# victorramirez952/tomography_3d_reconstructor

Hardware: NVIDIA B200
Metric: Gvoxels/s mask-stack->mesh+volume (higher is better)
Workload: dtype u8 -> bit-packed u32 (topology), f64 field taps -> f32 vertices

## Files before the change

tomography_3d_reconstructor_b200/csrc/t3d_mc.cu:

```cuda
#include "mc_tables.h"
#include "mc33_tables.h"
#include "t3d.h"
#include "t3d_field.cuh"

__device__ __align__(16) const int8_t g_tri_table[256][T3D_MC_ROW] = {T3D_TRI_TABLE_ROWS};
static const int8_t h_tri_table[256][T3D_MC_ROW] = {T3D_TRI_TABLE_ROWS};

struct McLuts {
    uint8_t ntri[256];
};
#define MC_AMB 0x80u
__constant__ McLuts c_luts;

__device__ const int8_t g33_rows[T3D_MC33_NROWS][T3D_MC33_ROW] = {T3D_MC33_TRI_ROWS};
__device__ const uint8_t g33_ntri[T3D_MC33_NROWS] = {T3D_MC33_NTRI_VALUES};
__device__ const uint16_t g33_base[256] = {T3D_MC33_BASE_VALUES};
__device__ const uint8_t g33_k[256] = {T3D_MC33_K_VALUES};
__device__ const uint8_t g33_faces[256][6] = {T3D_MC33_FACES_VALUES};
__device__ const unsigned long long g33_need[256] = {T3D_MC33_NEED_VALUES};
__device__ const uint8_t g33_pol[256] = {T3D_MC33_POL_VALUES};
__device__ const int8_t g33_sign[256] = {T3D_MC33_SIGN_VALUES};
__device__ const uint8_t g33_cyc[6][4] = {T3D_MC33_FACE_CYCLE_VALUES};
static const uint16_t h33_base[256] = {T3D_MC33_BASE_VALUES};

// ... 277 lines not shown
            int z, y;
            const WordMasks m = load_masks(g, row, w, z, y);
            int delta = 0;
            for (uint32_t a = m.act; a;) {
                const int b = __ffs(a) - 1;
                a &= a - 1;
                const int cs = cube_case(m, b);
                const uint32_t c = c_luts.ntri[cs];
                if (!(c & MC_AMB)) continue;
                delta += (int)g33_ntri[mc33_resolve(fld, z, y, (w << 5) + b, cs)] - (int)(c & 0x7fu);
                ++na;
            }
            aw_cnt[3 * (int64_t)n_active + k] += (uint32_t)delta;
        };
        const int64_t n4 = ((uintptr_t)aw_idx & 15) ? 0 : (n >> 2), stride = (int64_t)gridDim.x * blockDim.x, t0 = (int64_t)blockIdx.x * blockDim.x + threadIdx.x;
        for (int64_t c = t0; c < n4; c += stride) {
            const uint4 v = reinterpret_cast<const uint4*>(aw_idx)[c];
            if (!((v.x | v.y | v.z | v.w) & AW_AMB)) continue;
            if (v.x & AW_AMB) fix_word(4 * c, v.x);
            if (v.y & AW_AMB) fix_word(4 * c + 1, v.y);
            if (v.z & AW_AMB) fix_word(4 * c + 2, v.z);
            if (v.w & AW_AMB) fix_word(4 * c + 3, v.w);
        }
        for (int64_t k = 4 * n4 + t0; k < n; k += stride) {
            const uint32_t iraw = aw_idx[k];
            if (iraw & AW_AMB) fix_word(k, iraw);
        }
        if (na) atomicAdd(n_ambiguous, (unsigned long long)na);
    }
}

static unsigned amb_grid(uint32_t n) { const unsigned want = (n + 127) / 128, cap = (unsigned)T3D_NUM_SMS * 8; return want < cap ? (want ? want : 1) : cap; }

struct EmitArgs {
    Grid g;
    McField fld;
    const uint32_t* ballots;
    const uint32_t* chunkbase;
    const uint32_t* aw_idx;
    const uint32_t* aw_base;
    uint32_t cap_active;
    const unsigned long long* sizes;
    uint32_t cap_verts, cap_faces;
    unsigned long long* vkeys;
    int32_t* faces;
};

__device__ __forceinline__ uint32_t active_rank(const EmitArgs& a, uint32_t row, int w)
{
    const int64_t c = (int64_t)row * a.g.ncr + (w >> 5);
    return a.chunkbase[c] + __popc(a.ballots[c] & ((1u << (w & 31)) - 1u));
}

__device__ __forceinline__ uint32_t lt_mask(int b) { return b >= 32 ? 0xffffffffu : ((1u << b) - 1u); }

__device__ __forceinline__ unsigned long long vkey(int axis, int z, int y, int x)
{
    return (unsigned long long)axis | ((unsigned long long)x << 2) | ((unsigned long long)y << 22) | ((unsigned long long)z << 42);
}

template <int PARTS, int AMB>
__global__ void __launch_bounds__(128) k_mc_emit(EmitArgs a)
{
    __shared__ __align__(16) int8_t s_tri[256][T3D_MC_ROW];
    __shared__ uint32_t s_base[12][128];
    __shared__ uint32_t s_mask[12][128];
    __shared__ uint32_t s_next[4][128];
    if (AMB == 1) {
        int any = 0;
        uint32_t nw_ = a.cap_active;
        if (a.sizes[0] < nw_) nw_ = (uint32_t)a.sizes[0];
        for (uint32_t k = blockIdx.x * blockDim.x + threadIdx.x; k < nw_; k += gridDim.x * blockDim.x) any |= (int)(a.aw_idx[k] >> 31);
        if (!__syncthreads_or(any)) return;
    }
    if (PARTS & 2) {
        const int4* src = reinterpret_cast<const int4*>(&g_tri_table[0][0]);
        int4* dst = reinterpret_cast<int4*>(&s_tri[0][0]);
        for (int i = threadIdx.x; i < 256; i += blockDim.x) {
            dst[i] = src[i];
            if (c_luts.ntri[i] & MC_AMB) s_tri[i][T3D_MC_ROW - 1] = -2;
        }
        __syncthreads();
    }
    const uint32_t tid = threadIdx.x;
    uint32_t n_words = a.cap_active;
    if (a.sizes[0] < n_words) n_words = (uint32_t)a.sizes[0];
    const uint32_t offY = (uint32_t)a.sizes[1], offZ = (uint32_t)(a.sizes[1] + a.sizes[2]);
    if (a.sizes[1] + a.sizes[2] + a.sizes[3] > a.cap_verts || a.sizes[4] > a.cap_faces) return;
    auto emit_word = [&](const uint32_t k, const uint32_t iraw) {
    const uint32_t i = iraw & AW_MASK;
    const uint32_t row = i / (uint32_t)a.g.nws;
    const int w = (int)(i - row * (uint32_t)a.g.nws);
    int z, y;
    const WordMasks m = load_masks(a.g, row, w, z, y);
    const int64_t NA = a.cap_active;
    const uint32_t bX00 = a.aw_base[k], bY0 = offY + a.aw_base[NA + k], bZ0 = offZ + a.aw_base[2 * NA + k];
    uint32_t pT = a.aw_base[3 * NA + k];
    const int x0 = w << 5;

    if (PARTS & 1) {
        uint32_t id = bX00;
        for (uint32_t q = m.X00; q;) { const int b = __ffs(q) - 1; q &= q - 1; a.vkeys[id++] = vkey(2, z, y, x0 + b); }
        id = bY0;
        for (uint32_t q = m.Y0; q;) { const int b = __ffs(q) - 1; q &= q - 1; a.vkeys[id++] = vkey(1, z, y, x0 + b); }
        id = bZ0;
        for (uint32_t q = m.Z0; q;) { const int b = __ffs(q) - 1; q &= q - 1; a.vkeys[id++] = vkey(0, z, y, x0 + b); }
    }
    if (!(PARTS & 2) || !m.act) return;
    if (AMB == 0 && (iraw & AW_AMB)) return;

    const uint32_t Hs = (uint32_t)a.g.Hs;
    uint32_t bX01 = 0, bX10 = 0, bX11 = 0, bY1 = 0, bZ1 = 0;
    if (m.X01 | m.Z1) {
        const uint32_t r = active_rank(a, row + 1, w);
        bX01 = a.aw_base[r];
        bZ1 = offZ + a.aw_base[2 * NA + r];
    }
    if (m.X10 | m.Y1) {
        const uint32_t r = active_rank(a, row + Hs, w);
        bX10 = a.aw_base[r];
        bY1 = offY + a.aw_base[NA + r];
    }
    if (m.X11) bX11 = a.aw_base[active_rank(a, row + Hs + 1, w)];
    uint32_t nY0 = 0, nY1 = 0, nZ0 = 0, nZ1 = 0;
    if ((m.act >> 31) & 1u) {
        const uint32_t v1 = (m.a00 >> 31) & 1u, v2 = (m.a01 >> 31) & 1u, v5 = (m.a10 >> 31) & 1u, v6 = (m.a11 >> 31) & 1u;
        if (v1 != v2) nY0 = offY + a.aw_base[NA + active_rank(a, row, w + 1)];
        if (v5 != v6) nY1 = offY + a.aw_base[NA + active_rank(a, row + Hs, w + 1)];
        if (v1 != v5) nZ0 = offZ + a.aw_base[2 * NA + active_rank(a, row, w + 1)];
        if (v2 != v6) nZ1 = offZ + a.aw_base[2 * NA + active_rank(a, row + 1, w + 1)];
    }
    s_base[0][tid] = bX00; s_mask[0][tid] = m.X00;
    s_base[1][tid] = bY0;  s_mask[1][tid] = m.Y0;
    s_base[2][tid] = bX01; s_mask[2][tid] = m.X01;
    s_base[3][tid] = bY0;  s_mask[3][tid] = m.Y0;
    s_base[4][tid] = bX10; s_mask[4][tid] = m.X10;
    s_base[5][tid] = bY1;  s_mask[5][tid] = m.Y1;
    s_base[6][tid] = bX11; s_mask[6][tid] = m.X11;
    s_base[7][tid] = bY1;  s_mask[7][tid] = m.Y1;
    s_base[8][tid] = bZ0;  s_mask[8][tid] = m.Z0;
    s_base[9][tid] = bZ0;  s_mask[9][tid] = m.Z0;
    s_base[10][tid] = bZ1; s_mask[10][tid] = m.Z1;
    s_base[11][tid] = bZ1; s_mask[11][tid] = m.Z1;
    s_next[0][tid] = nY0; s_next[1][tid] = nY1; s_next[2][tid] = nZ0; s_next[3][tid] = nZ1;

    auto vertex_id = [&](int b, int e) -> uint32_t {
        const uint32_t at_next = (0x622u >> e) & 1u;
        uint32_t id = s_base[e][tid] + __popc(s_mask[e][tid] & (at_next ? lt_mask(b + 1) : lt_mask(b)));
        if (b == 31 && at_next) id = s_next[((e >> 2) & 1) + 2 * ((e >> 3) & 1) + ((e >> 3) & 1) * ((e >> 1) & 1)][tid];
        return id;
    };
    auto emit_classic = [&](int b, int cs) {
        const int4 trow = *reinterpret_cast<const int4*>(s_tri[cs]);
        const uint32_t tw[4] = {(uint32_t)trow.x, (uint32_t)trow.y, (uint32_t)trow.z, (uint32_t)trow.w};
        auto edge_at = [&](int t) -> int { return (int)(int8_t)((tw[t >> 2] >> ((t & 3) * 8)) & 0xffu); };
        for (int t = 0; t < 15; t += 3) {
            const int e0 = edge_at(t);
            if (e0 < 0) break;
            uint32_t vid[3];
#pragma unroll
            for (int c = 0; c < 3; ++c) vid[c] = vertex_id(b, (c == 0) ? e0 : edge_at(t + c));
            int32_t* f = a.faces + 3 * (int64_t)pT;
            f[0] = (int32_t)vid[2]; f[1] = (int32_t)vid[1]; f[2] = (int32_t)vid[0];
            ++pT;
        }
    };
    if constexpr (AMB == 0) {
        for (uint32_t q = m.act; q;) {
            const int b = __ffs(q) - 1;
            q &= q - 1;
            emit_classic(b, cube_case(m, b));
        }
    } else {
    for (uint32_t q = m.act; q;) {
        const int b = __ffs(q) - 1;
        q &= q - 1;
        const int cs = cube_case(m, b);
        if ((uint8_t)s_tri[cs][T3D_MC_ROW - 1] != 0xfeu) { emit_classic(b, cs); continue; }
        const int r = mc33_resolve(a.fld, z, y, x0 + b, cs);
        const int8_t* row = g33_rows[r];
        const int n3 = 3 * (int)g33_ntri[r];
        for (int t = 0; t < n3; t += 3) {
            int32_t* f = a.faces + 3 * (int64_t)pT;
            f[0] = (int32_t)vertex_id(b, row[t + 2]); f[1] = (int32_t)vertex_id(b, row[t + 1]); f[2] = (int32_t)vertex_id(b, row[t]);
            ++pT;
        }
    }
    }
    };
    if (AMB == 1) {
        for (uint32_t k = blockIdx.x * blockDim.x + tid; k < n_words; k += gridDim.x * blockDim.x) {
            const uint32_t iraw = a.aw_idx[k];
            if (iraw & AW_AMB) emit_word(k, iraw);
        }
    } else {
        const uint32_t k = blockIdx.x * blockDim.x + tid;
        if (k < n_words) emit_word(k, a.aw_idx[k]);
    }
}

struct VertexArgs {
    OccView occ;
    const float* field;
    double level;
    const unsigned long long* vkeys;
    int x_off;
    int z_offset;
    float shift;
    const double* cum;
    const double* adj;
    int n_cum;
    double mm_y, mm_x;
    int scale_f64;
    float* verts;
};

template <int AXIS>
__device__ __forceinline__ void vertex_body(const VertexArgs& p, const ZLut& zlut, uint32_t id)
{
    const unsigned long long key = p.vkeys[id];
    const int x = (int)((key >> 2) & 0xfffffu) - p.x_off, y = (int)((key >> 22) & 0xfffffu), z = (int)(key >> 42);
    float fa, fb;
    if (p.field) {
        const int64_t i = ((int64_t)z * p.occ.H + y) * p.occ.W + x;
        fa = p.field[i];
        fb = p.field[i + (AXIS == 0 ? (int64_t)p.occ.H * p.occ.W : AXIS == 1 ? p.occ.W : 1)];
    } else {
        edge_field_values<AXIS>(p.occ, zlut, z, y, x, fa, fb);
    }
    const double va = (double)fa - p.level, vb = (double)fb - p.level;
    const double wa = __ddiv_rn(1.0, __dadd_rn(MC33_EPS, fabs(va)));
    const double wb = __ddiv_rn(1.0, __dadd_rn(MC33_EPS, fabs(vb)));
    const double frac = __ddiv_rn(wb, __dadd_rn(wa, wb));
    double pz = (double)(z + p.z_offset), py = (double)y, px = (double)x;
    if (AXIS == 0) pz = __dadd_rn(pz, frac); else if (AXIS == 1) py = __dadd_rn(py, frac); else px = __dadd_rn(px, frac);
    float fz = __fsub_rn(__double2float_rn(pz), p.shift);
    float fy = __fsub_rn(__double2float_rn(py), p.shift);
    float fx = __fsub_rn(__double2float_rn(px), p.shift);
    if (p.n_cum > 0) {
        if (fz < 0.0f) fz = 0.0f;
        else if (fz >= (float)(p.n_cum - 1)) fz = __double2float_rn(p.cum[p.n_cum - 1]);
        else {
            const float fl = floorf(fz);
            const int lo = (int)fl;
            const float fr = __fsub_rn(fz, fl);
            const int ai = min(lo, p.n_cum - 2);
            fz = __double2float_rn(__dadd_rn(p.cum[lo], __dmul_rn((double)fr, p.adj[ai])));
        }
    }
    if (p.scale_f64) {
        fy = __double2float_rn(__dmul_rn((double)fy, p.mm_y));
        fx = __double2float_rn(__dmul_rn((double)fx, p.mm_x));
    } else {
        fy = __fmul_rn(fy, __double2float_rn(p.mm_y));
        fx = __fmul_rn(fx, __double2float_rn(p.mm_x));
    }
    float* o = p.verts + 3 * (int64_t)id;
    o[0] = fz; o[1] = fy; o[2] = fx;
}

__global__ void __launch_bounds__(128) k_mc_vertices_all(VertexArgs p, const unsigned long long* __restrict__ sizes, uint32_t cap_verts,
                                                         int which)
{
    __shared__ ZLut zlut;
    fill_zlut(p.occ, zlut);
    __syncthreads();
    const unsigned long long nx = sizes[1], ny = sizes[2], nz = sizes[3];
    if (nx + ny + nz > cap_verts) return;
    uint32_t t = blockIdx.x * blockDim.x + threadIdx.x;
    if (which & 1) {
        if (t < nx) { vertex_body<2>(p, zlut, t); return; }
        t -= (uint32_t)nx;
    }
    if (which & 2) {
        if (t < ny) { vertex_body<1>(p, zlut, (uint32_t)nx + t); return; }
        t -= (uint32_t)ny;
    }
    if ((which & 4) && t < nz) vertex_body<0>(p, zlut, (uint32_t)(nx + ny) + t);
}

static int make_grid(Grid& g, const void* sign_bits, int Zs, int Hs, int Ws, int z_begin, int z_end, const char* who)
{
    if (Zs <= 0 || Hs <= 0 || Ws <= 0) { t3d_set_error("%s: empty volume", who); return 2; }
    if (z_end < 0 || z_end > Zs) z_end = Zs;
    if (z_begin < 0 || z_begin >= z_end) { t3d_set_error("%s: empty plane range", who); return 2; }
    g.z_begin = z_begin; g.z_end = z_end;
    g.sign = (const uint32_t*)sign_bits;
    g.Zs = Zs; g.Hs = Hs; g.Ws = Ws; g.nws = t3d_wpr(Ws);
    g.ncr = (g.nws + 31) >> 5;
    g.n_rows = (uint32_t)((int64_t)Zs * Hs);
    g.n_words = (int64_t)Zs * Hs * g.nws;
    if (g.n_words >= ((int64_t)1 << 31)) { t3d_set_error("%s: more than 2^31 words in one device slab", who); return 2; }
    return 0;
}
// ... 36 lines not shown
    T3D_CHECK_LAUNCH("t3d_mc_words_dev");
    t3d_count_launches(3);
    return 0;
}

extern "C" int t3d_mc_words_dev(const void* sign_bits, int Zs, int Hs, int Ws, int z_begin, int z_end, const void* ballots_u32,
                                const void* chunkbase_u32, uint32_t cap_active, const void* sizes_u64, void* aw_idx_u32,
                                void* aw_cnt_u32, void* n_ambiguous_u64, const t3d_mc_field* mc_field, void* stream)
{
    return mc_words_dev_impl(mc_field_from_abi(mc_field), sign_bits, Zs, Hs, Ws, z_begin, z_end, ballots_u32, chunkbase_u32, cap_active,
                             sizes_u64, aw_idx_u32, aw_cnt_u32, n_ambiguous_u64, stream);
}

static int mc_emit_dev_impl(const McField& fld, const void* sign_bits, int Zs, int Hs, int Ws, int z_begin, int z_end,
                            const void* ballots_u32, const void* chunkbase_u32, const void* aw_idx_u32, const void* aw_base_u32,
                            uint32_t cap_active, const void* sizes_u64, uint32_t cap_verts, uint32_t cap_faces, void* vkeys_u64,
                            void* faces_i32, int parts, void* stream)
{
    EmitArgs a;
    if (int rc = make_grid(a.g, sign_bits, Zs, Hs, Ws, z_begin, z_end, "t3d_mc_emit_dev")) return rc;
    if (ensure_luts()) return 1;
    if (cap_active == 0) return 0;
    a.fld = fld;
    a.ballots = (const uint32_t*)ballots_u32;
    a.chunkbase = (const uint32_t*)chunkbase_u32;
    a.aw_idx = (const uint32_t*)aw_idx_u32;
    a.aw_base = (const uint32_t*)aw_base_u32;
    a.cap_active = cap_active;
    a.sizes = (const unsigned long long*)sizes_u64;
    a.cap_verts = cap_verts;
    a.cap_faces = cap_faces;
    a.vkeys = (unsigned long long*)vkeys_u64;
    a.faces = (int32_t*)faces_i32;
    const unsigned ge = (cap_active + 127) / 128;
    int launches = 1;
    if ((parts & 3) == 1) k_mc_emit<1, 0><<<ge, 128, 0, (cudaStream_t)stream>>>(a);
    else if ((parts & 3) == 2) {
        k_mc_emit<2, 0><<<ge, 128, 0, (cudaStream_t)stream>>>(a);
        k_mc_emit<2, 1><<<amb_grid(cap_active), 128, 0, (cudaStream_t)stream>>>(a);
        launches = 2;
    } else k_mc_emit<3, 2><<<ge, 128, 0, (cudaStream_t)stream>>>(a);
    T3D_CHECK_LAUNCH("t3d_mc_emit_dev");
    t3d_count_launches(launches);
    return 0;
}

extern "C" int t3d_mc_emit_dev(const void* sign_bits, int Zs, int Hs, int Ws, int z_begin, int z_end, const void* ballots_u32,
                               const void* chunkbase_u32, const void* aw_idx_u32, const void* aw_base_u32, uint32_t cap_active,
                               const void* sizes_u64, uint32_t cap_verts, uint32_t cap_faces, void* vkeys_u64, void* faces_i32,
                               int parts, const t3d_mc_field* mc_field, void* stream)
{
    return mc_emit_dev_impl(mc_field_from_abi(mc_field), sign_bits, Zs, Hs, Ws, z_begin, z_end, ballots_u32, chunkbase_u32, aw_idx_u32,
                            aw_base_u32, cap_active, sizes_u64, cap_verts, cap_faces, vkeys_u64, faces_i32, parts, stream);
}

int t3d_mc_words_view_dev(const OccView& view, int x_off, const void* sign_bits, int Zs, int Hs, int Ws, int z_begin, int z_end,
                          const void* ballots_u32, const void* chunkbase_u32, uint32_t cap_active, const void* sizes_u64,
                          void* aw_idx_u32, void* aw_cnt_u32, void* n_ambiguous_u64, void* stream)
{
    McField f;
    f.occ = view; f.field = nullptr; f.level = 0.5; f.x_off = x_off; f.mode = 1;
    return mc_words_dev_impl(f, sign_bits, Zs, Hs, Ws, z_begin, z_end, ballots_u32, chunkbase_u32, cap_active, sizes_u64, aw_idx_u32,
                             aw_cnt_u32, n_ambiguous_u64, stream);
}

int t3d_mc_emit_view_dev(const OccView& view, int x_off, const void* sign_bits, int Zs, int Hs, int Ws, int z_begin, int z_end,
                         const void* ballots_u32, const void* chunkbase_u32, const void* aw_idx_u32, const void* aw_base_u32,
                         uint32_t cap_active, const void* sizes_u64, uint32_t cap_verts, uint32_t cap_faces, void* vkeys_u64,
                         void* faces_i32, int parts, void* stream)
{
    McField f;
    f.occ = view; f.field = nullptr; f.level = 0.5; f.x_off = x_off; f.mode = 1;
    return mc_emit_dev_impl(f, sign_bits, Zs, Hs, Ws, z_begin, z_end, ballots_u32, chunkbase_u32, aw_idx_u32, aw_base_u32, cap_active,
                            sizes_u64, cap_verts, cap_faces, vkeys_u64, faces_i32, parts, stream);
}

// ... 77 lines not shown
```

tomography_3d_reconstructor_b200/csrc/t3d_field.cuh:

```cuda
#pragma once
#include "t3d_common.cuh"

struct OccView {
    const uint32_t* bits;
    int Z, H, W, nw;
    int rs;
    long long ps;
    int pad;
    int Zp, Hp, Wp;
    int gaussian;
    double w0, w1, w2;
};

__device__ __forceinline__ int reflect_idx(int i, int n)
{
    if (i >= 0 && i < n) return i;
    if (n == 1) return 0;
    const int period = 2 * n;
    i %= period;
    if (i < 0) i += period;
    return i < n ? i : period - 1 - i;
}

__device__ __forceinline__ uint32_t pbit(const OccView& v, int zp, int yp, int xp)
// ... 66 lines not shown
{
    const int z = zp - v.pad, y = yp - v.pad;
    if (z < 0 || z >= v.Z || y < 0 || y >= v.H || wp < 0) return 0u;
    const uint32_t* row = v.bits + (z * v.ps + (long long)y * v.rs);
    const uint32_t cur = (wp < v.nw) ? row[wp] : 0u;
    if (!v.pad) return cur;
    const uint32_t prev = (wp - 1 >= 0 && wp - 1 < v.nw) ? row[wp - 1] : 0u;
    return (cur << 1) | (prev >> 31);
}


__device__ __forceinline__ uint32_t get6(const OccView& v, int zp, int yp, int xs)
{
    const int z = zp - v.pad, y = yp - v.pad;
    if (z < 0 || z >= v.Z || y < 0 || y >= v.H) return 0u;
    const uint32_t* row = v.bits + (z * v.ps + (long long)y * v.rs);
    if (xs >= 0 && xs + 5 < v.Wp) {
        const int ox = xs - v.pad;
        const int w = ox >> 5, sh = ox & 31;
        const uint32_t lo = (w >= 0 && w < v.nw) ? row[w] : 0u;
        const uint32_t hi = (sh > 26 && w + 1 >= 0 && w + 1 < v.nw) ? row[w + 1] : 0u;
        const unsigned long long win = (unsigned long long)lo | ((unsigned long long)hi << 32);
        return (uint32_t)(win >> sh) & 63u;
    }
    uint32_t r = 0;
#pragma unroll
    for (int k = 0; k < 6; ++k) {
        const int ox = reflect_idx(xs + k, v.Wp) - v.pad;
        if (ox >= 0 && ox < v.W) r |= ((row[ox >> 5] >> (ox & 31)) & 1u) << k;
    }
    return r;
}

struct ZLut {
    double z[32];
    uint32_t spread[64];
};

__device__ __forceinline__ void fill_zlut(const OccView& v, ZLut& L)
{
    const int i = threadIdx.x;
    if (i < 32) {
        const int c = i >> 4, n2 = (i >> 2) & 3, n1 = i & 3;
        double t = __dmul_rn((double)c, v.w0);
        t = __dadd_rn(t, __dmul_rn((double)n2, v.w2));
        t = __dadd_rn(t, __dmul_rn((double)n1, v.w1));
        L.z[i] = t;
    }
    if (i < 64) {
        uint32_t r = 0;
        for (int k = 0; k < 6; ++k) r |= ((uint32_t)(i >> k) & 1u) << (5 * k);
        L.spread[i] = r;
    }
}

template <int AXIS>
__device__ __forceinline__ void edge_field_values(const OccView& v, const ZLut& L, int z, int y, int x, float& fa, float& fb)
{
    if (!v.gaussian) {
        fa = pbit(v, z, y, x) ? 1.0f : 0.0f;
        fb = pbit(v, z + (AXIS == 0), y + (AXIS == 1), x + (AXIS == 2)) ? 1.0f : 0.0f;
        return;
    }
    constexpr int NZ = 5 + (AXIS == 0), NY = 5 + (AXIS == 1), NE = 1 + (AXIS == 0);
    uint32_t idx[NE][NY];
#pragma unroll
    for (int e = 0; e < NE; ++e)
#pragma unroll
        for (int dy = 0; dy < NY; ++dy) idx[e][dy] = 0u;
    auto add_plane = [&](int dy, int dz, uint32_t six) {
        const uint32_t s = L.spread[six];
#pragma unroll
        for (int e = 0; e < NE; ++e) {
            const int j = dz - e;
            if (j < 0 || j > 4) continue;
            idx[e][dy] += s << (j == 2 ? 4 : (j == 0 || j == 4) ? 2 : 0);
        }
    };
    const int oz0 = z - 2 - v.pad, oy0 = y - 2 - v.pad, ox0 = x - 2 - v.pad;
    if (oz0 >= 0 && oz0 + NZ <= v.Z && oy0 >= 0 && oy0 + NY <= v.H && ox0 >= 0 && ox0 + 6 <= v.W) {
        const int w = ox0 >> 5, sh = ox0 & 31;
        const bool two = sh > 26;
        const uint32_t* p = v.bits + (oz0 * v.ps + (long long)oy0 * v.rs) + w;
        const long long dzs = v.ps;
#pragma unroll
        for (int dy = 0; dy < NY; ++dy) {
#pragma unroll
            for (int dz = 0; dz < NZ; ++dz) {
                const uint32_t* q = p + dz * dzs + dy * v.rs;
                const uint32_t lo = q[0], hi = two ? q[1] : 0u;
                add_plane(dy, dz, __funnelshift_r(lo, hi, sh) & 63u);
            }
        }
    } else {
#pragma unroll
        for (int dy = 0; dy < NY; ++dy) {
            const int yr = reflect_idx(y - 2 + dy, v.Hp);
#pragma unroll
            for (int dz = 0; dz < NZ; ++dz) add_plane(dy, dz, get6(v, reflect_idx(z - 2 + dz, v.Zp), yr, x - 2));
        }
    }
    auto zpass = [&](int dy, int k, int e) -> double { return L.z[(idx[e][dy] >> (5 * k)) & 31u]; };
    if (AXIS == 2) {
        double Y[6];
#pragma unroll
        for (int k = 0; k < 6; ++k)
            Y[k] = corr5(zpass(0, k, 0), zpass(1, k, 0), zpass(2, k, 0), zpass(3, k, 0), zpass(4, k, 0), v.w0, v.w1, v.w2);
        fa = __double2float_rn(corr5(Y[0], Y[1], Y[2], Y[3], Y[4], v.w0, v.w1, v.w2));
        fb = __double2float_rn(corr5(Y[1], Y[2], Y[3], Y[4], Y[5], v.w0, v.w1, v.w2));
    } else if (AXIS == 1) {
        double Ya[5], Yb[5];
#pragma unroll
        for (int k = 0; k < 5; ++k) {
            double A[6];
#pragma unroll
            for (int dy = 0; dy < 6; ++dy) A[dy] = zpass(dy, k, 0);
            Ya[k] = corr5(A[0], A[1], A[2], A[3], A[4], v.w0, v.w1, v.w2);
            Yb[k] = corr5(A[1], A[2], A[3], A[4], A[5], v.w0, v.w1, v.w2);
        }
        fa = __double2float_rn(corr5(Ya[0], Ya[1], Ya[2], Ya[3], Ya[4], v.w0, v.w1, v.w2));
        fb = __double2float_rn(corr5(Yb[0], Yb[1], Yb[2], Yb[3], Yb[4], v.w0, v.w1, v.w2));
    } else {
#pragma unroll
        for (int e = 0; e < 2; ++e) {
            double Y[5];
#pragma unroll
            for (int k = 0; k < 5; ++k)
                Y[k] = corr5(zpass(0, k, e), zpass(1, k, e), zpass(2, k, e), zpass(3, k, e), zpass(4, k, e), v.w0, v.w1, v.w2);
            const float f = __double2float_rn(corr5(Y[0], Y[1], Y[2], Y[3], Y[4], v.w0, v.w1, v.w2));
            if (e == 0) fa = f; else fb = f;
        }
    }
}

static inline OccView t3d_make_view(const void* occ_bits, int Z, int H, int W, int pad, int gaussian, const double* w3)
{
    OccView v;
    v.bits = (const uint32_t*)occ_bits;
    v.Z = Z; v.H = H; v.W = W; v.nw = t3d_wpr(W);
    v.rs = v.nw; v.ps = (long long)H * v.nw;
    v.pad = pad ? 1 : 0;
    v.Zp = Z + 2 * v.pad; v.Hp = H + 2 * v.pad; v.Wp = W + 2 * v.pad;
    v.gaussian = gaussian ? 1 : 0;
    v.w0 = w3 ? w3[0] : 0x1.92b965ef5aaeep-1;
    v.w1 = w3 ? w3[1] : 0x1.b405b9842b206p-4;
    v.w2 = w3 ? w3[2] : 0x1.14aebe6a24088p-12;
    return v;
}

static inline OccView t3d_make_view_strided(const void* origin, int Z, int H, int W, int row_stride, long long plane_stride, int pad,
                                            int gaussian, const double* w3)
{
    OccView v = t3d_make_view(origin, Z, H, W, pad, gaussian, w3);
    v.rs = row_stride; v.ps = plane_stride;
    return v;
}

int t3d_mc_vertices_view_dev(const OccView& view, int x_off, const void* vkeys_u64, const void* sizes_u64, uint32_t cap_verts,
                             int unpad_shift, int z_offset, const void* cum_f64, const void* adj_f64, int n_cum, double mm_per_pixel_y,
                             double mm_per_pixel_x, int scale_in_f64, int which_blocks, void* verts_f32, void* stream);
int t3d_mc_words_view_dev(const OccView& view, int x_off, const void* sign_bits, int Zs, int Hs, int Ws, int z_begin, int z_end,
                          const void* ballots_u32, const void* chunkbase_u32, uint32_t cap_active, const void* sizes_u64,
                          void* aw_idx_u32, void* aw_cnt_u32, void* n_ambiguous_u64, void* stream);
int t3d_mc_emit_view_dev(const OccView& view, int x_off, const void* sign_bits, int Zs, int Hs, int Ws, int z_begin, int z_end,
                         const void* ballots_u32, const void* chunkbase_u32, const void* aw_idx_u32, const void* aw_base_u32,
// ... 3 lines not shown
```

Measured before the change: 858.0.

## Split MC emit into warp-cooperative key and face kernels with per-warp work lists

The monolithic templated emit kernel becomes separate kernels for vertex keys, classic faces, and ambiguous faces. Key and face emission now run a warp prefix scan to flatten per-word bit work into a shared list, so lanes share the writes instead of each thread serially looping over up to 32 bits. The aim is to remove warp divergence and load imbalance and to get more coalesced output stores. In exchange it adds shuffle scans, shared staging, and extra launches when both parts run, and the previous combined parts=3 mode becomes separate passes.

```diff
diff --git a/tomography_3d_reconstructor_b200/csrc/t3d_mc.cu b/tomography_3d_reconstructor_b200/csrc/t3d_mc.cu
--- a/tomography_3d_reconstructor_b200/csrc/t3d_mc.cu
+++ b/tomography_3d_reconstructor_b200/csrc/t3d_mc.cu
@@ -333,6 +333,9 @@
 
 static unsigned amb_grid(uint32_t n) { const unsigned want = (n + 127) / 128, cap = (unsigned)T3D_NUM_SMS * 8; return want < cap ? (want ? want : 1) : cap; }
 
+#define EMIT_WORDS 128
+#define EMIT_LIST 256
+
 struct EmitArgs {
     Grid g;
     McField fld;
@@ -347,6 +350,12 @@
     int32_t* faces;
 };
 
+__device__ __forceinline__ uint32_t emit_words(const EmitArgs& a)
+{
+    if (a.sizes[1] + a.sizes[2] + a.sizes[3] > a.cap_verts || a.sizes[4] > a.cap_faces) return 0;
+    return a.sizes[0] < a.cap_active ? (uint32_t)a.sizes[0] : a.cap_active;
+}
+
 __device__ __forceinline__ uint32_t active_rank(const EmitArgs& a, uint32_t row, int w)
 {
     const int64_t c = (int64_t)row * a.g.ncr + (w >> 5);
@@ -360,56 +369,73 @@
     return (unsigned long long)axis | ((unsigned long long)x << 2) | ((unsigned long long)y << 22) | ((unsigned long long)z << 42);
 }
 
-template <int PARTS, int AMB>
-__global__ void __launch_bounds__(128) k_mc_emit(EmitArgs a)
-{
-    __shared__ __align__(16) int8_t s_tri[256][T3D_MC_ROW];
-    __shared__ uint32_t s_base[12][128];
-    __shared__ uint32_t s_mask[12][128];
-    __shared__ uint32_t s_next[4][128];
-    if (AMB == 1) {
-        int any = 0;
-        uint32_t nw_ = a.cap_active;
-        if (a.sizes[0] < nw_) nw_ = (uint32_t)a.sizes[0];
-        for (uint32_t k = blockIdx.x * blockDim.x + threadIdx.x; k < nw_; k += gridDim.x * blockDim.x) any |= (int)(a.aw_idx[k] >> 31);
-        if (!__syncthreads_or(any)) return;
-    }
-    if (PARTS & 2) {
-        const int4* src = reinterpret_cast<const int4*>(&g_tri_table[0][0]);
-        int4* dst = reinterpret_cast<int4*>(&s_tri[0][0]);
-        for (int i = threadIdx.x; i < 256; i += blockDim.x) {
-            dst[i] = src[i];
-            if (c_luts.ntri[i] & MC_AMB) s_tri[i][T3D_MC_ROW - 1] = -2;
-        }
-        __syncthreads();
-    }
-    const uint32_t tid = threadIdx.x;
-    uint32_t n_words = a.cap_active;
-    if (a.sizes[0] < n_words) n_words = (uint32_t)a.sizes[0];
+template <typename T>
+__device__ __forceinline__ T warp_exclusive_scan(T v, T& total)
+{
+    const int lane = threadIdx.x & 31;
+    T x = v;
+#pragma unroll
+    for (int d = 1; d < 32; d <<= 1) {
+        const T y = __shfl_up_sync(0xffffffffu, x, d);
+        if (lane >= d) x += y;
+    }
+    total = __shfl_sync(0xffffffffu, x, 31);
+    return x - v;
+}
+
+__global__ void __launch_bounds__(EMIT_WORDS) k_mc_keys(EmitArgs a)
+{
+    __shared__ unsigned long long s_key[EMIT_WORDS];
+    __shared__ uint16_t s_list[EMIT_WORDS / 32][EMIT_LIST];
+    const uint32_t n_words = emit_words(a), tid = threadIdx.x, lane = tid & 31, k = blockIdx.x * EMIT_WORDS + tid, kw = k - lane;
+    if (kw >= n_words) return;
+    uint32_t qX = 0, qY = 0, qZ = 0;
+    if (k < n_words) {
+        const uint32_t i = a.aw_idx[k] & AW_MASK;
+        const uint32_t row = i / (uint32_t)a.g.nws;
+        const int w = (int)(i - row * (uint32_t)a.g.nws);
+        int z, y;
+        const WordMasks m = load_masks(a.g, row, w, z, y);
+        qX = m.X00; qY = m.Y0; qZ = m.Z0;
+        s_key[tid] = vkey(0, z, y, w << 5);
+    }
+    unsigned long long tot;
+    const unsigned long long o = warp_exclusive_scan<unsigned long long>(
+        (unsigned long long)__popc(qX) | ((unsigned long long)__popc(qY) << 21) | ((unsigned long long)__popc(qZ) << 42), tot);
+    const uint32_t nx = (uint32_t)(tot & 0x1fffffu), ny = (uint32_t)((tot >> 21) & 0x1fffffu), n = nx + ny + (uint32_t)(tot >> 42);
+    uint32_t pX = (uint32_t)(o & 0x1fffffu), pY = nx + (uint32_t)((o >> 21) & 0x1fffffu), pZ = nx + ny + (uint32_t)(o >> 42);
+    const int64_t NA = a.cap_active;
     const uint32_t offY = (uint32_t)a.sizes[1], offZ = (uint32_t)(a.sizes[1] + a.sizes[2]);
-    if (a.sizes[1] + a.sizes[2] + a.sizes[3] > a.cap_verts || a.sizes[4] > a.cap_faces) return;
-    auto emit_word = [&](const uint32_t k, const uint32_t iraw) {
-    const uint32_t i = iraw & AW_MASK;
-    const uint32_t row = i / (uint32_t)a.g.nws;
-    const int w = (int)(i - row * (uint32_t)a.g.nws);
-    int z, y;
-    const WordMasks m = load_masks(a.g, row, w, z, y);
+    const uint32_t dX = a.aw_base[kw], dY = offY + a.aw_base[NA + kw] - nx, dZ = offZ + a.aw_base[2 * NA + kw] - nx - ny;
+    uint16_t* list = s_list[tid >> 5];
+    const unsigned long long* key = s_key + (tid & ~31u);
+    for (uint32_t r0 = 0; r0 < n; r0 += EMIT_LIST) {
+        const uint32_t r1 = r0 + EMIT_LIST;
+        for (; qX && pX < r1; qX &= qX - 1) list[pX++ - r0] = (uint16_t)(lane << 5 | (__ffs(qX) - 1));
+        for (; qY && pY < r1; qY &= qY - 1) list[pY++ - r0] = (uint16_t)(lane << 5 | (__ffs(qY) - 1));
+        for (; qZ && pZ < r1; qZ &= qZ - 1) list[pZ++ - r0] = (uint16_t)(lane << 5 | (__ffs(qZ) - 1));
+        __syncwarp();
+        for (uint32_t j = r0 + lane; j < min(n, r1); j += 32) {
+            const uint32_t e = list[j - r0];
+            const int axis = j < nx ? 2 : (j < nx + ny ? 1 : 0);
+            a.vkeys[j + (axis == 2 ? dX : (axis == 1 ? dY : dZ))] = key[e >> 5] | ((unsigned long long)(e & 31u) << 2) | (unsigned long long)axis;
+        }
+        __syncwarp();
+    }
+}
+
+struct EmitTables {
+    uint32_t base[12][EMIT_WORDS];
+    uint32_t mask[12][EMIT_WORDS];
+    uint32_t next[4][EMIT_WORDS];
+};
+
+__device__ __forceinline__ void word_tables(const EmitArgs& a, EmitTables& s, int slot, const WordMasks& m, uint32_t row, int w,
+                                            uint32_t k)
+{
     const int64_t NA = a.cap_active;
+    const uint32_t offY = (uint32_t)a.sizes[1], offZ = (uint32_t)(a.sizes[1] + a.sizes[2]);
     const uint32_t bX00 = a.aw_base[k], bY0 = offY + a.aw_base[NA + k], bZ0 = offZ + a.aw_base[2 * NA + k];
-    uint32_t pT = a.aw_base[3 * NA + k];
-    const int x0 = w << 5;
-
-    if (PARTS & 1) {
-        uint32_t id = bX00;
-        for (uint32_t q = m.X00; q;) { const int b = __ffs(q) - 1; q &= q - 1; a.vkeys[id++] = vkey(2, z, y, x0 + b); }
-        id = bY0;
-        for (uint32_t q = m.Y0; q;) { const int b = __ffs(q) - 1; q &= q - 1; a.vkeys[id++] = vkey(1, z, y, x0 + b); }
-        id = bZ0;
-        for (uint32_t q = m.Z0; q;) { const int b = __ffs(q) - 1; q &= q - 1; a.vkeys[id++] = vkey(0, z, y, x0 + b); }
-    }
-    if (!(PARTS & 2) || !m.act) return;
-    if (AMB == 0 && (iraw & AW_AMB)) return;
-
     const uint32_t Hs = (uint32_t)a.g.Hs;
     uint32_t bX01 = 0, bX10 = 0, bX11 = 0, bY1 = 0, bZ1 = 0;
     if (m.X01 | m.Z1) {
@@ -431,72 +457,160 @@
         if (v1 != v5) nZ0 = offZ + a.aw_base[2 * NA + active_rank(a, row, w + 1)];
         if (v2 != v6) nZ1 = offZ + a.aw_base[2 * NA + active_rank(a, row + 1, w + 1)];
     }
-    s_base[0][tid] = bX00; s_mask[0][tid] = m.X00;
-    s_base[1][tid] = bY0;  s_mask[1][tid] = m.Y0;
-    s_base[2][tid] = bX01; s_mask[2][tid] = m.X01;
-    s_base[3][tid] = bY0;  s_mask[3][tid] = m.Y0;
-    s_base[4][tid] = bX10; s_mask[4][tid] = m.X10;
-    s_base[5][tid] = bY1;  s_mask[5][tid] = m.Y1;
-    s_base[6][tid] = bX11; s_mask[6][tid] = m.X11;
-    s_base[7][tid] = bY1;  s_mask[7][tid] = m.Y1;
-    s_base[8][tid] = bZ0;  s_mask[8][tid] = m.Z0;
-    s_base[9][tid] = bZ0;  s_mask[9][tid] = m.Z0;
-    s_base[10][tid] = bZ1; s_mask[10][tid] = m.Z1;
-    s_base[11][tid] = bZ1; s_mask[11][tid] = m.Z1;
-    s_next[0][tid] = nY0; s_next[1][tid] = nY1; s_next[2][tid] = nZ0; s_next[3][tid] = nZ1;
-
-    auto vertex_id = [&](int b, int e) -> uint32_t {
-        const uint32_t at_next = (0x622u >> e) & 1u;
-        uint32_t id = s_base[e][tid] + __popc(s_mask[e][tid] & (at_next ? lt_mask(b + 1) : lt_mask(b)));
-        if (b == 31 && at_next) id = s_next[((e >> 2) & 1) + 2 * ((e >> 3) & 1) + ((e >> 3) & 1) * ((e >> 1) & 1)][tid];
-        return id;
-    };
-    auto emit_classic = [&](int b, int cs) {
-        const int4 trow = *reinterpret_cast<const int4*>(s_tri[cs]);
-        const uint32_t tw[4] = {(uint32_t)trow.x, (uint32_t)trow.y, (uint32_t)trow.z, (uint32_t)trow.w};
-        auto edge_at = [&](int t) -> int { return (int)(int8_t)((tw[t >> 2] >> ((t & 3) * 8)) & 0xffu); };
-        for (int t = 0; t < 15; t += 3) {
-            const int e0 = edge_at(t);
-            if (e0 < 0) break;
-            uint32_t vid[3];
+    s.base[0][slot] = bX00; s.mask[0][slot] = m.X00;
+    s.base[1][slot] = bY0;  s.mask[1][slot] = m.Y0;
+    s.base[2][slot] = bX01; s.mask[2][slot] = m.X01;
+    s.base[3][slot] = bY0;  s.mask[3][slot] = m.Y0;
+    s.base[4][slot] = bX10; s.mask[4][slot] = m.X10;
+    s.base[5][slot] = bY1;  s.mask[5][slot] = m.Y1;
+    s.base[6][slot] = bX11; s.mask[6][slot] = m.X11;
+    s.base[7][slot] = bY1;  s.mask[7][slot] = m.Y1;
+    s.base[8][slot] = bZ0;  s.mask[8][slot] = m.Z0;
+    s.base[9][slot] = bZ0;  s.mask[9][slot] = m.Z0;
+    s.base[10][slot] = bZ1; s.mask[10][slot] = m.Z1;
+    s.base[11][slot] = bZ1; s.mask[11][slot] = m.Z1;
+    s.next[0][slot] = nY0; s.next[1][slot] = nY1; s.next[2][slot] = nZ0; s.next[3][slot] = nZ1;
+}
+
+__device__ __forceinline__ uint32_t vertex_id(const EmitTables& s, int slot, int b, int e)
+{
+    const uint32_t at_next = (0x622u >> e) & 1u;
+    uint32_t id = s.base[e][slot] + __popc(s.mask[e][slot] & (at_next ? lt_mask(b + 1) : lt_mask(b)));
+    if (b == 31 && at_next) id = s.next[((e >> 2) & 1) + 2 * ((e >> 3) & 1) + ((e >> 3) & 1) * ((e >> 1) & 1)][slot];
+    return id;
+}
+
+__device__ __forceinline__ int4 tri_row(int cs) { return __ldg(reinterpret_cast<const int4*>(g_tri_table[cs])); }
+
+__device__ __forceinline__ uint32_t row_triangles(int4 r)
+{
+    return (uint32_t)(__popc(__vcmpges4(r.x, 0)) + __popc(__vcmpges4(r.y, 0)) + __popc(__vcmpges4(r.z, 0)) + __popc(__vcmpges4(r.w, 0))) / 24u;
+}
+
+__device__ __forceinline__ uint32_t emit_classic(const EmitArgs& a, const EmitTables& s, int slot, int b, int4 trow, uint32_t pT)
+{
+    const uint32_t tw[4] = {(uint32_t)trow.x, (uint32_t)trow.y, (uint32_t)trow.z, (uint32_t)trow.w};
+    auto edge_at = [&](int t) -> int { return (int)(int8_t)((tw[t >> 2] >> ((t & 3) * 8)) & 0xffu); };
+    for (int t = 0; t < 15; t += 3) {
+        const int e0 = edge_at(t);
+        if (e0 < 0) break;
+        uint32_t vid[3];
 #pragma unroll
-            for (int c = 0; c < 3; ++c) vid[c] = vertex_id(b, (c == 0) ? e0 : edge_at(t + c));
-            int32_t* f = a.faces + 3 * (int64_t)pT;
-            f[0] = (int32_t)vid[2]; f[1] = (int32_t)vid[1]; f[2] = (int32_t)vid[0];
-            ++pT;
-        }
-    };
-    if constexpr (AMB == 0) {
+        for (int c = 0; c < 3; ++c) vid[c] = vertex_id(s, slot, b, (c == 0) ? e0 : edge_at(t + c));
+        int32_t* f = a.faces + 3 * (int64_t)pT;
+        f[0] = (int32_t)vid[2]; f[1] = (int32_t)vid[1]; f[2] = (int32_t)vid[0];
+        ++pT;
+    }
+    return pT;
+}
+
+__global__ void __launch_bounds__(EMIT_WORDS) k_mc_faces(EmitArgs a)
+{
+    __shared__ EmitTables s;
+    __shared__ uint32_t s_pT[EMIT_WORDS];
+    __shared__ uint32_t s_list[EMIT_WORDS / 32][EMIT_LIST];
+    const uint32_t n_words = emit_words(a), tid = threadIdx.x, lane = tid & 31, k = blockIdx.x * EMIT_WORDS + tid;
+    if (k - lane >= n_words) return;
+    WordMasks m = {};
+    uint32_t act = 0;
+    if (k < n_words) {
+        const uint32_t iraw = a.aw_idx[k];
+        if (!(iraw & AW_AMB)) {
+            const uint32_t i = iraw & AW_MASK;
+            const uint32_t row = i / (uint32_t)a.g.nws;
+            const int w = (int)(i - row * (uint32_t)a.g.nws);
+            int z, y;
+            m = load_masks(a.g, row, w, z, y);
+            act = m.act;
+            if (act) {
+                word_tables(a, s, tid, m, row, w, k);
+                s_pT[tid] = a.aw_base[3 * (int64_t)a.cap_active + k];
+            }
+        }
+    }
+    uint32_t total;
+    uint32_t pos = warp_exclusive_scan<uint32_t>(__popc(act), total);
+    uint32_t* list = s_list[tid >> 5];
+    const uint32_t slot0 = tid & ~31u;
+    uint32_t rel = 0;
+    for (uint32_t r0 = 0; r0 < total; r0 += EMIT_LIST) {
+        for (; act && pos < r0 + EMIT_LIST; ++pos) {
+            const int b = __ffs(act) - 1;
+            act &= act - 1;
+            const int cs = cube_case(m, b);
+            list[pos - r0] = lane << 21 | (uint32_t)b << 16 | (uint32_t)cs << 8 | rel;
+            rel += row_triangles(tri_row(cs));
+        }
+        __syncwarp();
+        const uint32_t n = min(total - r0, (uint32_t)EMIT_LIST);
+        for (uint32_t j = lane; j < n; j += 32) {
+            const uint32_t e = list[j];
+            const int slot = (int)(slot0 + (e >> 21));
+            const int cs = (int)((e >> 8) & 0xffu);
+            emit_classic(a, s, slot, (int)((e >> 16) & 31u), tri_row(cs), s_pT[slot] + (e & 0xffu));
+        }
+        __syncwarp();
+    }
+}
+
+__global__ void __launch_bounds__(EMIT_WORDS) k_mc_faces_amb(EmitArgs a)
+{
+    __shared__ __align__(16) int8_t s_tri[256][T3D_MC_ROW];
+    __shared__ EmitTables s;
+    const uint32_t n_words = emit_words(a), stride = gridDim.x * blockDim.x, t0 = blockIdx.x * blockDim.x + threadIdx.x;
+    const uint32_t n4 = ((uintptr_t)a.aw_idx & 15) ? 0 : (n_words >> 2);
+    const uint4* idx4 = reinterpret_cast<const uint4*>(a.aw_idx);
+    int any = 0;
+    for (uint32_t c = t0; c < n4; c += stride) {
+        const uint4 v = idx4[c];
+        any |= (int)((v.x | v.y | v.z | v.w) >> 31);
+    }
+    for (uint32_t k = 4 * n4 + t0; k < n_words; k += stride) any |= (int)(a.aw_idx[k] >> 31);
+    if (!__syncthreads_or(any)) return;
+    for (int i = threadIdx.x; i < 256; i += blockDim.x) {
+        reinterpret_cast<int4*>(&s_tri[0][0])[i] = reinterpret_cast<const int4*>(&g_tri_table[0][0])[i];
+        if (c_luts.ntri[i] & MC_AMB) s_tri[i][T3D_MC_ROW - 1] = -2;
+    }
+    __syncthreads();
+    const int tid = threadIdx.x;
+    auto emit_word = [&](const uint32_t k, const uint32_t iraw) {
+        const uint32_t i = iraw & AW_MASK;
+        const uint32_t row = i / (uint32_t)a.g.nws;
+        const int w = (int)(i - row * (uint32_t)a.g.nws);
+        int z, y;
+        const WordMasks m = load_masks(a.g, row, w, z, y);
+        word_tables(a, s, tid, m, row, w, k);
+        uint32_t pT = a.aw_base[3 * (int64_t)a.cap_active + k];
         for (uint32_t q = m.act; q;) {
             const int b = __ffs(q) - 1;
             q &= q - 1;
-            emit_classic(b, cube_case(m, b));
-        }
-    } else {
-    for (uint32_t q = m.act; q;) {
-        const int b = __ffs(q) - 1;
-        q &= q - 1;
-        const int cs = cube_case(m, b);
-        if ((uint8_t)s_tri[cs][T3D_MC_ROW - 1] != 0xfeu) { emit_classic(b, cs); continue; }
-        const int r = mc33_resolve(a.fld, z, y, x0 + b, cs);
-        const int8_t* row = g33_rows[r];
-        const int n3 = 3 * (int)g33_ntri[r];
-        for (int t = 0; t < n3; t += 3) {
-            int32_t* f = a.faces + 3 * (int64_t)pT;
-            f[0] = (int32_t)vertex_id(b, row[t + 2]); f[1] = (int32_t)vertex_id(b, row[t + 1]); f[2] = (int32_t)vertex_id(b, row[t]);
-            ++pT;
-        }
-    }
-    }
+            const int cs = cube_case(m, b);
+            if ((uint8_t)s_tri[cs][T3D_MC_ROW - 1] != 0xfeu) {
+                pT = emit_classic(a, s, tid, b, *reinterpret_cast<const int4*>(s_tri[cs]), pT);
+                continue;
+            }
+            const int r = mc33_resolve(a.fld, z, y, (w << 5) + b, cs);
+            const int8_t* trow = g33_rows[r];
+            const int n3 = 3 * (int)g33_ntri[r];
+            for (int t = 0; t < n3; t += 3) {
+                int32_t* f = a.faces + 3 * (int64_t)pT;
+                f[0] = (int32_t)vertex_id(s, tid, b, trow[t + 2]); f[1] = (int32_t)vertex_id(s, tid, b, trow[t + 1]);
+                f[2] = (int32_t)vertex_id(s, tid, b, trow[t]);
+                ++pT;
+            }
+        }
     };
-    if (AMB == 1) {
-        for (uint32_t k = blockIdx.x * blockDim.x + tid; k < n_words; k += gridDim.x * blockDim.x) {
-            const uint32_t iraw = a.aw_idx[k];
-            if (iraw & AW_AMB) emit_word(k, iraw);
-        }
-    } else {
-        const uint32_t k = blockIdx.x * blockDim.x + tid;
-        if (k < n_words) emit_word(k, a.aw_idx[k]);
+    for (uint32_t c = t0; c < n4; c += stride) {
+        const uint4 v = idx4[c];
+        if (!((v.x | v.y | v.z | v.w) & AW_AMB)) continue;
+        if (v.x & AW_AMB) emit_word(4 * c, v.x);
+        if (v.y & AW_AMB) emit_word(4 * c + 1, v.y);
+        if (v.z & AW_AMB) emit_word(4 * c + 2, v.z);
+        if (v.w & AW_AMB) emit_word(4 * c + 3, v.w);
+    }
+    for (uint32_t k = 4 * n4 + t0; k < n_words; k += stride) {
+        const uint32_t iraw = a.aw_idx[k];
+        if (iraw & AW_AMB) emit_word(k, iraw);
     }
 }
 
@@ -663,16 +777,16 @@
     a.cap_faces = cap_faces;
     a.vkeys = (unsigned long long*)vkeys_u64;
     a.faces = (int32_t*)faces_i32;
-    const unsigned ge = (cap_active + 127) / 128;
-    int launches = 1;
-    if ((parts & 3) == 1) k_mc_emit<1, 0><<<ge, 128, 0, (cudaStream_t)stream>>>(a);
-    else if ((parts & 3) == 2) {
-        k_mc_emit<2, 0><<<ge, 128, 0, (cudaStream_t)stream>>>(a);
-        k_mc_emit<2, 1><<<amb_grid(cap_active), 128, 0, (cudaStream_t)stream>>>(a);
-        launches = 2;
-    } else k_mc_emit<3, 2><<<ge, 128, 0, (cudaStream_t)stream>>>(a);
+    cudaStream_t st = (cudaStream_t)stream;
+    const unsigned ge = (cap_active + EMIT_WORDS - 1) / EMIT_WORDS;
+    const int p = (parts & 3) ? (parts & 3) : 3;
+    if (p & 1) k_mc_keys<<<ge, EMIT_WORDS, 0, st>>>(a);
+    if (p & 2) {
+        k_mc_faces<<<ge, EMIT_WORDS, 0, st>>>(a);
+        k_mc_faces_amb<<<amb_grid(cap_active), EMIT_WORDS, 0, st>>>(a);
+    }
     T3D_CHECK_LAUNCH("t3d_mc_emit_dev");
-    t3d_count_launches(launches);
+    t3d_count_launches((p & 1) + ((p & 2) ? 2 : 0));
     return 0;
 }
 
```

Result: faster. 871.0, median of 6 (+1.5%).

## Restructure Gaussian edge-field taps: arithmetic spread, rotated row loads, noinline border path

Applied to the files above, without the earlier changes.

Replaces the shared-memory spread lookup with an arithmetic bit-spread (multiply-and-mask) and computes the per-plane weighted sums directly from a gathered 2D array of 6-bit rows. Interior rows are loaded in a rotated order keyed on oy0 mod NY and then un-rotated with selects, apparently to spread loads across different addresses/banks. The reflect-padded border path moves into a separate noinline function to cut register pressure in the hot path, and the vertex kernel gets launch_bounds(128,8) to raise occupancy. The risks are extra select instructions for the un-rotation, possible register spills under the tighter bound, and call overhead on border voxels.

```diff
diff --git a/.bench_libs/prof.py b/.bench_libs/prof.py
--- /dev/null
+++ b/.bench_libs/prof.py
@@ -0,0 +1,28 @@
+import sys, os, json, collections
+sys.path.insert(0, os.getcwd()); sys.path.insert(0, os.path.join(os.getcwd(), "tools"))
+import torch
+from torch.profiler import profile, ProfilerActivity
+import vertex_bench as vb
+from bench import PHYS, THRESHOLD, make_phantom_u8, side_counts
+from tomography_3d_reconstructor_b200 import _lib, pipeline
+builds = {"base": vb.load_build(".bench_libs/base.so"), "new": vb.load_build("tomography_3d_reconstructor_b200/libt3d.so")}
+Z, H, W = 512, 1024, 1024
+masks = make_phantom_u8(Z, H, W, 0, Z, torch.device("cuda", 0))
+sides = side_counts(Z); phys = (PHYS["total_depth_mm"], PHYS["x_length_mm"], PHYS["y_length_mm"])
+plans = {}
+for b, lib in builds.items():
+    _lib._lib = lib; pipeline._plans.clear(); pipeline._hints.clear()
+    for _ in range(3): pipeline.reconstruct_fused(masks, THRESHOLD, sides, *phys)
+    plans[b] = pipeline._plans[pipeline.plan_key(masks, THRESHOLD, sides, *phys)]
+for b in builds:
+    for _ in range(5): plans[b].graph.replay()
+    torch.cuda.synchronize()
+    with profile(activities=[ProfilerActivity.CUDA]) as prof:
+        for _ in range(10): plans[b].graph.replay()
+        torch.cuda.synchronize()
+    agg = collections.defaultdict(float)
+    ev = [e for e in prof.events() if e.device_type.name == "CUDA"]
+    t0 = min(e.time_range.start for e in ev); t1 = max(e.time_range.end for e in ev)
+    for e in ev: agg[e.name[:60]] += e.device_time / 10 if hasattr(e, "device_time") else e.cuda_time / 10
+    print(b, "span per step us", (t1 - t0) / 10)
+    for k, v in sorted(agg.items(), key=lambda kv: -kv[1])[:14]: print("  %8.1f  %s" % (v, k))
diff --git a/tomography_3d_reconstructor_b200/csrc/t3d_field.cuh b/tomography_3d_reconstructor_b200/csrc/t3d_field.cuh
--- a/tomography_3d_reconstructor_b200/csrc/t3d_field.cuh
+++ b/tomography_3d_reconstructor_b200/csrc/t3d_field.cuh
@@ -122,82 +122,65 @@
     return r;
 }
 
+__device__ __forceinline__ double zpass_value(double w0, double w1, double w2, int i)
+{
+    const int c = i >> 4, n2 = (i >> 2) & 3, n1 = i & 3;
+    double t = __dmul_rn((double)c, w0);
+    t = __dadd_rn(t, __dmul_rn((double)n2, w2));
+    t = __dadd_rn(t, __dmul_rn((double)n1, w1));
+    return t;
+}
+
 struct ZLut {
     double z[32];
     uint32_t spread[64];
 };
 
+__device__ __forceinline__ uint32_t spread6(uint32_t six)
+{
+    return ((((six & 0x38u) << 12) | (six & 7u)) * 0x111u) & 0x2108421u;
+}
+
 __device__ __forceinline__ void fill_zlut(const OccView& v, ZLut& L)
 {
     const int i = threadIdx.x;
-    if (i < 32) {
-        const int c = i >> 4, n2 = (i >> 2) & 3, n1 = i & 3;
-        double t = __dmul_rn((double)c, v.w0);
-        t = __dadd_rn(t, __dmul_rn((double)n2, v.w2));
-        t = __dadd_rn(t, __dmul_rn((double)n1, v.w1));
-        L.z[i] = t;
-    }
-    if (i < 64) {
-        uint32_t r = 0;
-        for (int k = 0; k < 6; ++k) r |= ((uint32_t)(i >> k) & 1u) << (5 * k);
-        L.spread[i] = r;
-    }
+    if (i < 32) L.z[i] = zpass_value(v.w0, v.w1, v.w2, i);
+    if (i < 64) L.spread[i] = spread6(i);
 }
 
 template <int AXIS>
-__device__ __forceinline__ void edge_field_values(const OccView& v, const ZLut& L, int z, int y, int x, float& fa, float& fb)
-{
-    if (!v.gaussian) {
-        fa = pbit(v, z, y, x) ? 1.0f : 0.0f;
-        fb = pbit(v, z + (AXIS == 0), y + (AXIS == 1), x + (AXIS == 2)) ? 1.0f : 0.0f;
-        return;
-    }
+__device__ __forceinline__ float2 edge_field_from_rows(const OccView& v, const ZLut& L, const uint32_t (&r)[5 + (AXIS == 0)][5 + (AXIS == 1)],
+                                                       int rot)
+{
     constexpr int NZ = 5 + (AXIS == 0), NY = 5 + (AXIS == 1), NE = 1 + (AXIS == 0);
+    uint32_t fetched[NE][NY];
+#pragma unroll
+    for (int j = 0; j < NY; ++j) {
+        uint32_t s[NZ];
+#pragma unroll
+        for (int dz = 0; dz < NZ; ++dz) s[dz] = spread6(r[dz][j]);
+#pragma unroll
+        for (int e = 0; e < NE; ++e) fetched[e][j] = ((s[e] + s[e + 4]) << 2) + s[e + 1] + s[e + 3] + (s[e + 2] << 4);
+    }
     uint32_t idx[NE][NY];
 #pragma unroll
     for (int e = 0; e < NE; ++e)
 #pragma unroll
-        for (int dy = 0; dy < NY; ++dy) idx[e][dy] = 0u;
-    auto add_plane = [&](int dy, int dz, uint32_t six) {
-        const uint32_t s = L.spread[six];
-#pragma unroll
-        for (int e = 0; e < NE; ++e) {
-            const int j = dz - e;
-            if (j < 0 || j > 4) continue;
-            idx[e][dy] += s << (j == 2 ? 4 : (j == 0 || j == 4) ? 2 : 0);
-        }
-    };
-    const int oz0 = z - 2 - v.pad, oy0 = y - 2 - v.pad, ox0 = x - 2 - v.pad;
-    if (oz0 >= 0 && oz0 + NZ <= v.Z && oy0 >= 0 && oy0 + NY <= v.H && ox0 >= 0 && ox0 + 6 <= v.W) {
-        const int w = ox0 >> 5, sh = ox0 & 31;
-        const bool two = sh > 26;
-        const uint32_t* p = v.bits + (oz0 * v.ps + (long long)oy0 * v.rs) + w;
-        const long long dzs = v.ps;
-#pragma unroll
         for (int dy = 0; dy < NY; ++dy) {
-#pragma unroll
-            for (int dz = 0; dz < NZ; ++dz) {
-                const uint32_t* q = p + dz * dzs + dy * v.rs;
-                const uint32_t lo = q[0], hi = two ? q[1] : 0u;
-                add_plane(dy, dz, __funnelshift_r(lo, hi, sh) & 63u);
-            }
-        }
-    } else {
-#pragma unroll
-        for (int dy = 0; dy < NY; ++dy) {
-            const int yr = reflect_idx(y - 2 + dy, v.Hp);
-#pragma unroll
-            for (int dz = 0; dz < NZ; ++dz) add_plane(dy, dz, get6(v, reflect_idx(z - 2 + dz, v.Zp), yr, x - 2));
-        }
-    }
+            uint32_t w = fetched[e][dy];
+#pragma unroll
+            for (int c = 1; c < NY; ++c) w = rot == c ? fetched[e][(dy + c) % NY] : w;
+            idx[e][dy] = w;
+        }
     auto zpass = [&](int dy, int k, int e) -> double { return L.z[(idx[e][dy] >> (5 * k)) & 31u]; };
+    float2 f;
     if (AXIS == 2) {
         double Y[6];
 #pragma unroll
         for (int k = 0; k < 6; ++k)
             Y[k] = corr5(zpass(0, k, 0), zpass(1, k, 0), zpass(2, k, 0), zpass(3, k, 0), zpass(4, k, 0), v.w0, v.w1, v.w2);
-        fa = __double2float_rn(corr5(Y[0], Y[1], Y[2], Y[3], Y[4], v.w0, v.w1, v.w2));
-        fb = __double2float_rn(corr5(Y[1], Y[2], Y[3], Y[4], Y[5], v.w0, v.w1, v.w2));
+        f.x = __double2float_rn(corr5(Y[0], Y[1], Y[2], Y[3], Y[4], v.w0, v.w1, v.w2));
+        f.y = __double2float_rn(corr5(Y[1], Y[2], Y[3], Y[4], Y[5], v.w0, v.w1, v.w2));
     } else if (AXIS == 1) {
         double Ya[5], Yb[5];
 #pragma unroll
@@ -208,19 +191,59 @@
             Ya[k] = corr5(A[0], A[1], A[2], A[3], A[4], v.w0, v.w1, v.w2);
             Yb[k] = corr5(A[1], A[2], A[3], A[4], A[5], v.w0, v.w1, v.w2);
         }
-        fa = __double2float_rn(corr5(Ya[0], Ya[1], Ya[2], Ya[3], Ya[4], v.w0, v.w1, v.w2));
-        fb = __double2float_rn(corr5(Yb[0], Yb[1], Yb[2], Yb[3], Yb[4], v.w0, v.w1, v.w2));
+        f.x = __double2float_rn(corr5(Ya[0], Ya[1], Ya[2], Ya[3], Ya[4], v.w0, v.w1, v.w2));
+        f.y = __double2float_rn(corr5(Yb[0], Yb[1], Yb[2], Yb[3], Yb[4], v.w0, v.w1, v.w2));
     } else {
+        float fe[2];
 #pragma unroll
         for (int e = 0; e < 2; ++e) {
             double Y[5];
 #pragma unroll
             for (int k = 0; k < 5; ++k)
                 Y[k] = corr5(zpass(0, k, e), zpass(1, k, e), zpass(2, k, e), zpass(3, k, e), zpass(4, k, e), v.w0, v.w1, v.w2);
-            const float f = __double2float_rn(corr5(Y[0], Y[1], Y[2], Y[3], Y[4], v.w0, v.w1, v.w2));
-            if (e == 0) fa = f; else fb = f;
-        }
-    }
+            fe[e] = __double2float_rn(corr5(Y[0], Y[1], Y[2], Y[3], Y[4], v.w0, v.w1, v.w2));
+        }
+        f.x = fe[0]; f.y = fe[1];
+    }
+    return f;
+}
+
+template <int AXIS>
+__device__ __noinline__ float2 edge_field_values_border(const OccView v, const ZLut& L, int z, int y, int x)
+{
+    constexpr int NZ = 5 + (AXIS == 0), NY = 5 + (AXIS == 1);
+    uint32_t r[NZ][NY];
+#pragma unroll
+    for (int dz = 0; dz < NZ; ++dz) {
+        const int zr = reflect_idx(z - 2 + dz, v.Zp);
+#pragma unroll
+        for (int dy = 0; dy < NY; ++dy) r[dz][dy] = get6(v, zr, reflect_idx(y - 2 + dy, v.Hp), x - 2);
+    }
+    return edge_field_from_rows<AXIS>(v, L, r, 0);
+}
+
+template <int AXIS>
+__device__ __forceinline__ float2 edge_field_values(const OccView& v, const ZLut& L, int z, int y, int x)
+{
+    if (!v.gaussian)
+        return make_float2(pbit(v, z, y, x) ? 1.0f : 0.0f, pbit(v, z + (AXIS == 0), y + (AXIS == 1), x + (AXIS == 2)) ? 1.0f : 0.0f);
+    constexpr int NZ = 5 + (AXIS == 0), NY = 5 + (AXIS == 1);
+    const int oz0 = z - 2 - v.pad, oy0 = y - 2 - v.pad, ox0 = x - 2 - v.pad;
+    if (!(oz0 >= 0 && oz0 + NZ <= v.Z && oy0 >= 0 && oy0 + NY <= v.H && ox0 >= 0 && ox0 + 6 <= v.W))
+        return edge_field_values_border<AXIS>(v, L, z, y, x);
+    const int sh = ox0 & 31;
+    const bool two = sh > 26;
+    const int rot = oy0 % NY;
+    const uint32_t* q = v.bits + (oz0 * v.ps + (long long)oy0 * v.rs) + (ox0 >> 5);
+    uint32_t r[NZ][NY];
+#pragma unroll
+    for (int j = 0; j < NY; ++j) {
+        const int dy = j >= rot ? j - rot : j - rot + NY;
+        const uint32_t* qr = q + (long long)dy * v.rs;
+#pragma unroll
+        for (int dz = 0; dz < NZ; ++dz, qr += v.ps) r[dz][j] = __funnelshift_r(qr[0], two ? qr[1] : 0u, sh) & 63u;
+    }
+    return edge_field_from_rows<AXIS>(v, L, r, rot);
 }
 
 static inline OccView t3d_make_view(const void* occ_bits, int Z, int H, int W, int pad, int gaussian, const double* w3)
diff --git a/tomography_3d_reconstructor_b200/csrc/t3d_mc.cu b/tomography_3d_reconstructor_b200/csrc/t3d_mc.cu
--- a/tomography_3d_reconstructor_b200/csrc/t3d_mc.cu
+++ b/tomography_3d_reconstructor_b200/csrc/t3d_mc.cu
@@ -527,7 +527,8 @@
         fa = p.field[i];
         fb = p.field[i + (AXIS == 0 ? (int64_t)p.occ.H * p.occ.W : AXIS == 1 ? p.occ.W : 1)];
     } else {
-        edge_field_values<AXIS>(p.occ, zlut, z, y, x, fa, fb);
+        const float2 f = edge_field_values<AXIS>(p.occ, zlut, z, y, x);
+        fa = f.x; fb = f.y;
     }
     const double va = (double)fa - p.level, vb = (double)fb - p.level;
     const double wa = __ddiv_rn(1.0, __dadd_rn(MC33_EPS, fabs(va)));
@@ -560,7 +561,7 @@
     o[0] = fz; o[1] = fy; o[2] = fx;
 }
 
-__global__ void __launch_bounds__(128) k_mc_vertices_all(VertexArgs p, const unsigned long long* __restrict__ sizes, uint32_t cap_verts,
+__global__ void __launch_bounds__(128, 8) k_mc_vertices_all(VertexArgs p, const unsigned long long* __restrict__ sizes, uint32_t cap_verts,
                                                          int which)
 {
     __shared__ ZLut zlut;
```

New measurement: 857.2 before, 878.7 after, median of 6. 2.5% higher.
